# simonhmartin/genomics_general

Measured on NVIDIA H100. Metric: sites/sec popgenWindows (pi+Fst+Dxy), higher is better.
Workload: dtype u8

## Files before the change

genomics_general_b200/csrc/k1.cu:

```cuda
#include <stdlib.h>

#include <algorithm>
#include <climits>
#include <cmath>
#include <type_traits>
#include <cub/cub.cuh>

#include "pgwin_internal.h"

namespace {

constexpr int K1_MAX_WARPS = 12;

enum { MODE_POPGEN = 0, MODE_ABBA = 1, MODE_COUNTS = 2, MODE_POPGEN_FREQ = 3, MODE_FOURPOP = 4 };

struct K1Params {
    const uint8_t* geno;
    const int32_t* pos;
    int64_t site_begin, site_end;
    int64_t num_tiles;
    int pitch, G, I, T, wpt, stages, tile_bytes, nw;
    const int32_t* ent_chunk;
    const uint4* ent_mask;
    int n_ent;
// ... 822 lines not shown
        if (lane == 0) mbar_arrive(&empty[stage]);
    }
    if (MODE != MODE_COUNTS) flush();
}


template <int P>
__device__ __forceinline__ void packed_walk(const K1Params& prm, int G, int gsub, int sl, uint32_t (&walk)[P]) {
#pragma unroll
    for (int X = 0; X < P; ++X) {
        const int n = prm.ent_hi[X] - prm.ent_lo[X];
        const int cnt = gsub < n ? (n - gsub + G - 1) / G : 0;
        const int first = prm.ent_lo[X] + (n > 0 ? (((sl >> 2) & 7) + gsub) % n : 0);
        walk[X] = (uint32_t)first | ((uint32_t)cnt << 16);
    }
}

template <int P>
struct ArrCounts {
    uint32_t nn[P], cc[P][4];
    __device__ __forceinline__ void set(int X, uint32_t p0, uint32_t p1) {
        const uint32_t m = p0 & 0xffffu, n1 = p0 >> 16, n2 = p1 & 0xffffu, n3 = p1 >> 16;
        nn[X] = m;
        cc[X][0] = m - n1 - n2 + n3;
        cc[X][1] = n1 - n3;
        cc[X][2] = n2 - n3;
        cc[X][3] = n3;
    }
    __device__ __forceinline__ uint32_t n(int X) const { return nn[X]; }
    __device__ __forceinline__ uint32_t c(int X, int a) const { return cc[X][a]; }
};
template <int P>
struct PkCounts {
    uint32_t p0[P], p1[P];
    __device__ __forceinline__ void set(int X, uint32_t a, uint32_t b) {
        p0[X] = a;
        p1[X] = b;
    }
    __device__ __forceinline__ uint32_t n(int X) const { return p0[X] & 0xffffu; }
    __device__ __forceinline__ uint32_t c(int X, int a) const {
        const uint32_t n1 = p0[X] >> 16, n2 = p1[X] & 0xffffu, n3 = p1[X] >> 16;
        return a == 0 ? (p0[X] & 0xffffu) - n1 - n2 + n3 : (a == 1 ? n1 - n3 : (a == 2 ? n2 - n3 : n3));
    }
};

template <int P, class W, class CT>
__device__ __forceinline__ void packed_counts(const K1Params& prm, const uint2* s_ent, const uint32_t* row, const W& walk,
                                              int G, int spw, CT& ct) {
    const int wd = prm.wd;
#pragma unroll
    for (int X = 0; X < P; ++X) {
        uint32_t a = 0u, a1 = 0u, a2 = 0u, a3 = 0u;
        const int lo = prm.ent_lo[X], span = prm.ent_hi[X] - lo;
        int e = (int)(walk[X] & 0xffffu);
        const int cnt = (int)(walk[X] >> 16);
        for (int k = 0; k < cnt; ++k) {
            const uint2 em = s_ent[e];
            const uint32_t m = row[em.x] & em.y;
            const uint32_t b0 = row[wd + em.x], b1 = row[2 * wd + em.x];
            a += __popc(m);
            a1 += __popc(m & b0);
            a2 += __popc(m & b1);
            a3 += __popc(m & b0 & b1);
            e += G;
            if (e >= lo + span) e -= span;
        }
        uint32_t p0 = a | (a1 << 16), p1 = a2 | (a3 << 16);
        for (int d = spw; d < 32; d <<= 1) {
            p0 += __shfl_xor_sync(0xffffffffu, p0, d);
            p1 += __shfl_xor_sync(0xffffffffu, p1, d);
        }
        ct.set(X, p0, p1);
    }
}

template <int P, bool ONE, class CT>
__device__ __forceinline__ void varied_counts(const K1Params& prm, const uint2* s_ent, const uint32_t* row, int nvar, int Gv,
                                              int gsub, int spv, CT& ct) {
    const int pn = prm.wd * nvar;
#pragma unroll
    for (int X = 0; X < P; ++X) {
        uint32_t a = 0u, a1 = 0u, a2 = 0u, a3 = 0u;
#pragma unroll 1
        for (int e = prm.ent_lo[X] + (ONE ? 0 : gsub); e < prm.ent_hi[X]; e += (ONE ? 1 : Gv)) {
            const uint2 em = s_ent[e];
            const uint32_t* w = row + em.x * nvar;
            const uint32_t m = w[0] & em.y;
            const uint32_t b0 = w[pn], b1 = w[2 * pn];
            a += __popc(m);
            a1 += __popc(m & b0);
            a2 += __popc(m & b1);
            a3 += __popc(m & b0 & b1);
        }
        uint32_t p0 = a | (a1 << 16), p1 = a2 | (a3 << 16);
        for (int d = spv; !ONE && d < 32; d <<= 1) {
            p0 += __shfl_xor_sync(0xffffffffu, p0, d);
            p1 += __shfl_xor_sync(0xffffffffu, p1, d);
        }
        ct.set(X, p0, p1);
    }
}

template <int P>
struct BitCounts {
    uint32_t k[P];
    const int* N;
    __device__ __forceinline__ void set(int X, uint32_t kx) { k[X] = kx; }
    __device__ __forceinline__ uint32_t n(int X) const { return (uint32_t)N[X]; }
    __device__ __forceinline__ uint32_t c(int X, int a) const { return a == 0 ? (uint32_t)N[X] - k[X] : (a == 1 ? k[X] : 0u); }
};

__device__ __forceinline__ void bmma_and_popc(int (&d)[4], uint32_t a0, uint32_t a1, uint32_t a2, uint32_t a3, uint2 b) {
    asm("mma.sync.aligned.m16n8k256.row.col.s32.b1.b1.s32.and.popc {%0, %1, %2, %3}, {%4, %5, %6, %7}, {%8, %9}, "
        "{%0, %1, %2, %3};"
        : "+r"(d[0]), "+r"(d[1]), "+r"(d[2]), "+r"(d[3])
        : "r"(a0), "r"(a1), "r"(a2), "r"(a3), "r"(b.x), "r"(b.y));
}

__device__ __forceinline__ int mma_row(int lane) { return (lane >> 2) + 8 * (lane & 3); }

template <int P>
__device__ __forceinline__ void varied_mma(const uint2* s_bf, const uint32_t* rows, int n1, int wd, int r, int lane,
                                           BitCounts<P>& ct) {
    static_assert(P <= 4, "one-plane rows: up to 4 (padded) populations");
    const int g = lane >> 2, t = lane & 3;
    const int j0 = min(r + g, n1 - 1), j1 = min(r + g + 8, n1 - 1), j2 = min(r + g + 16, n1 - 1), j3 = min(r + g + 24, n1 - 1);
    int d0[4] = {0, 0, 0, 0}, d1[4] = {0, 0, 0, 0};
    const uint32_t* w = rows + t * n1;
    for (int kb = 0; kb * 8 < wd; ++kb, w += 8 * n1) {
        const bool lo = kb * 8 + t < wd, hi = kb * 8 + 4 + t < wd;
        const uint32_t* v = w + 4 * n1;
        const uint2 b = s_bf[kb * 32 + lane];
        bmma_and_popc(d0, lo ? w[j0] : 0u, lo ? w[j1] : 0u, hi ? v[j0] : 0u, hi ? v[j1] : 0u, b);
        bmma_and_popc(d1, lo ? w[j2] : 0u, lo ? w[j3] : 0u, hi ? v[j2] : 0u, hi ? v[j3] : 0u, b);
    }
    const uint32_t pk[4] = {(uint32_t)d0[0] | (uint32_t)d0[1] << 16, (uint32_t)d0[2] | (uint32_t)d0[3] << 16,
                            (uint32_t)d1[0] | (uint32_t)d1[1] << 16, (uint32_t)d1[2] | (uint32_t)d1[3] << 16};
    uint32_t k01 = 0u, k23 = 0u;
#pragma unroll
    for (int j = 0; j < 4; ++j) {
        const int q = t ^ j;
        const uint32_t v = __shfl_xor_sync(0xffffffffu, (q & 2) ? ((q & 1) ? pk[3] : pk[2]) : ((q & 1) ? pk[1] : pk[0]), j);
        if (q == 0) k01 = v;
        if (q == 1) k23 = v;
    }
    ct.set(0, k01 & 0xffffu);
    ct.set(1, k01 >> 16);
    if constexpr (P > 2) {
        ct.set(2, k23 & 0xffffu);
        ct.set(3, k23 >> 16);
    }
}

template <int P, class CT>
__device__ __forceinline__ void packed_class(const K1Params& prm, bool owner, const CT& ct, bool& pres, bool& ragged) {
    bool allpres = true, allmiss = true;
#pragma unroll
    for (int X = 0; X < P; ++X) {
        allpres = allpres && (ct.n(X) == (uint32_t)prm.popN[X]);
        allmiss = allmiss && (ct.n(X) == 0u);
    }
    pres = owner && allpres;
    ragged = owner && !allpres && !allmiss;
}

template <int MODE, int P, class ACC, class CT>
__device__ __forceinline__ void packed_add(ACC& acc, bool pres, bool ragged, const CT& ct) {
    acc.i[0] += pres ? 1 : 0;
    acc.i[1] += ragged ? 1 : 0;
    const uint32_t f = pres ? 1u : 0u;
#pragma unroll
    for (int X = 0; X < P; ++X) {
        const uint32_t sq = ct.c(X, 0) * ct.c(X, 0) + ct.c(X, 1) * ct.c(X, 1) + ct.c(X, 2) * ct.c(X, 2) + ct.c(X, 3) * ct.c(X, 3);
        acc.u[X] += sq * f;
        if (MODE == MODE_POPGEN_FREQ) acc.u[P + P * (P - 1) / 2 + X] += (pres && sq != ct.n(X) * ct.n(X)) ? 1u : 0u;
    }
    int k = 0;
#pragma unroll
    for (int X = 0; X < P; ++X)
#pragma unroll
        for (int Y = X + 1; Y < P; ++Y) {
            const uint32_t cr = ct.c(X, 0) * ct.c(Y, 0) + ct.c(X, 1) * ct.c(Y, 1) + ct.c(X, 2) * ct.c(Y, 2) + ct.c(X, 3) * ct.c(Y, 3);
            acc.u[P + k] += cr * f;
            ++k;
        }
}

template <int MODE, int P, int NW, bool UNI = false>
__global__ void __launch_bounds__((NW + 1) * 32, 1) k1_site_pass_packed(const __grid_constant__ K1Params prm) {
    static_assert(MODE == MODE_POPGEN || MODE == MODE_POPGEN_FREQ, "packed site pass: popgen modes");
    constexpr int K1_THREADS = (NW + 1) * 32;
    constexpr int QI = ModeTraits<MODE, P>::QI, QU = ModeTraits<MODE, P>::QU;
    extern __shared__ __align__(128) uint8_t smem[];
    uint8_t* tiles = smem;
    uint64_t* full = reinterpret_cast<uint64_t*>(smem + (size_t)prm.stages * prm.tile_bytes);
    uint64_t* empty = full + 8;
    volatile int* s_issued = reinterpret_cast<volatile int*>(empty + 8);
    volatile uint32_t* s_nvar = reinterpret_cast<volatile uint32_t*>(s_issued + 8);
    volatile long long* s_site0 = reinterpret_cast<volatile long long*>(s_issued + 16);
    uint2* s_ent = reinterpret_cast<uint2*>(smem + (size_t)prm.stages * prm.tile_bytes + 256);
    uint2* s_bf = s_ent + prm.n_ent;

    const int tid = threadIdx.x, lane = tid & 31, warp = tid >> 5;
    const int b = blockIdx.x, B = gridDim.x;
    const int64_t t0 = (int64_t)b * prm.num_tiles / B, t1 = (int64_t)(b + 1) * prm.num_tiles / B;
    const int ntiles = (int)(t1 - t0);

    for (int e = tid; e < prm.n_ent; e += K1_THREADS) s_ent[e] = prm.word_ent[e];
    if constexpr (UNI && P < 8)
        for (int e = tid; e < (prm.wd + 7) / 8 * 32; e += K1_THREADS) s_bf[e] = prm.bit_frag[e];
    const int Gv = prm.uni_gv > 0 ? prm.uni_gv : prm.G;
    if (tid == 0) {
        for (int s = 0; s < prm.stages; ++s) {
            mbar_init(&full[s], 1);
            mbar_init(&empty[s], (uint32_t)prm.wpt);
        }
        *s_issued = 0;
        asm volatile("fence.mbarrier_init.release.cluster;" ::: "memory");
        asm volatile("fence.proxy.async.shared::cta;" ::: "memory");
    }
    __syncthreads();

    if (warp == NW) {
        if (UNI) k1_producer_uniform(prm, tiles, full, empty, s_issued, s_nvar, s_site0, ntiles, t0, lane);
        else if (lane == 0) k1_producer<MODE>(prm, tiles, full, empty, s_issued, ntiles, t0);
        return;
    }

    const int nteams = NW / prm.wpt;
    const int team = warp / prm.wpt, lw = warp % prm.wpt;

    Acc<QI, QU, 0> acc;
#pragma unroll
    for (int q = 0; q < QI; ++q) acc.i[q] = 0;
#pragma unroll
    for (int q = 0; q < QU; ++q) acc.u[q] = 0u;
    int since_flush = 0;
    int cur_seg = -1;
    int64_t seg_end = -1;
    const int seg_first = prm.cta_seg_first[b];
    const int64_t slot_base = prm.cta_slot_off[b];

    if constexpr (!UNI) {
        const int G = prm.G;
        const int spw = 32 / G;
        const int gsub = lane / spw;
        const int sl = lane % spw;
        const int sites_per_iter = prm.wpt * spw;
        uint32_t walk[P];
        packed_walk<P>(prm, G, gsub, sl, walk);

        for (int it = team; it < ntiles; it += nteams) {
            const int stage = it % prm.stages;
            if (lane == 0)
                while (atomicAdd(const_cast<int*>(s_issued), 0) <= it) __nanosleep(20);
            __syncwarp();
            mbar_wait(&full[stage], (uint32_t)((it / prm.stages) & 1));
            const uint8_t* tile = tiles + (size_t)stage * prm.tile_bytes;
            const int64_t tile_site0 = prm.site_begin + (t0 + it) * prm.T;

            for (int i = 0; i < prm.I; ++i) {
                const int slot = i * sites_per_iter + lw * spw + sl;
                const int64_t site = tile_site0 + slot;
                const bool valid = site < prm.site_end;
                const bool owner = valid && (gsub == 0);
                const uint32_t* row = reinterpret_cast<const uint32_t*>(tile + (size_t)(valid ? slot : 0) * prm.pitch);
                const int posv = owner ? reinterpret_cast<const int32_t*>(tile + (size_t)prm.T * prm.pitch)[slot] : 0;

                ArrCounts<P> ct;
                packed_counts<P>(prm, s_ent, row, walk, G, spw, ct);

                int sg = cur_seg;
                if (owner && site >= seg_end) sg = find_seg(prm.brk, prm.nseg, cur_seg + 1, site);
                if (__any_sync(0xffffffffu, sg != cur_seg)) {
                    warp_flush<QI, QU, 0>(acc, cur_seg, prm.part, slot_base, seg_first, warp, lane, NW);
                    since_flush = 0;
                    if (sg != cur_seg) {
                        cur_seg = sg;
                        seg_end = __ldg(prm.brk + sg + 1);
                    }
                }
                bool pres, ragged;
                packed_class<P>(prm, owner, ct, pres, ragged);
                if (++since_flush > prm.acc_limit) {
                    warp_flush<QI, QU, 0>(acc, cur_seg, prm.part, slot_base, seg_first, warp, lane, NW);
                    since_flush = 1;
                }
                acc.i[2] += (long long)posv;
                packed_add<MODE, P>(acc, pres, ragged, ct);
            }

            __syncwarp();
            if (lane == 0) mbar_arrive(&empty[stage]);
        }
    } else {
        const int spv = 32 / Gv, gsub = lane / spv, sl = lane % spv, wpt = prm.wpt;
        auto add_row = [&](int64_t site, bool owner, const auto& ct, bool back) {
            int sg = cur_seg;
            if (owner && site >= seg_end) sg = next_seg(prm.brk, prm.nseg, cur_seg + 1, site);
            else if (back && owner && site < __ldg(prm.brk + cur_seg)) sg = find_seg(prm.brk, cur_seg, 0, site);
            if (__any_sync(0xffffffffu, sg != cur_seg)) {
                warp_flush<QI, QU, 0>(acc, cur_seg, prm.part, slot_base, seg_first, warp, lane, NW);
                since_flush = 0;
                const int last = __reduce_max_sync(0xffffffffu, sg);
                const int to = owner ? sg : last;
                if (to != cur_seg) {
                    cur_seg = to;
                    seg_end = __ldg(prm.brk + to + 1);
                }
            }
            bool pres, ragged;
            packed_class<P>(prm, owner, ct, pres, ragged);
            if (++since_flush > prm.acc_limit) {
                warp_flush<QI, QU, 0>(acc, cur_seg, prm.part, slot_base, seg_first, warp, lane, NW);
                since_flush = 1;
            }
            packed_add<MODE, P>(acc, pres, ragged, ct);
        };

        for (int it = team; it < ntiles; it += nteams) {
            const int stage = it % prm.stages;
            if (lane == 0)
                while (atomicAdd(const_cast<int*>(s_issued), 0) <= it) __nanosleep(20);
            __syncwarp();
            mbar_wait(&full[stage], (uint32_t)((it / prm.stages) & 1));
            const uint8_t* tile = tiles + (size_t)stage * prm.tile_bytes;
            const int64_t tile_site0 = s_site0[stage];
            const uint32_t sizes = s_nvar[stage];
            const int n1 = (int)(sizes & 0xffffu), n3 = (int)(sizes >> 16);
            const uint16_t* s_slot = reinterpret_cast<const uint16_t*>(tile + (size_t)prm.row_cap * prm.pitch);
            const int rot = (int)((t0 + it) % wpt), nb1 = (n1 + 31) / 32;

            if constexpr (P < 8) {
                for (int r = ((lw - rot + wpt) % wpt) * 32; r < n1; r += wpt * 32) {
                    const int rw = r + mma_row(lane);
                    BitCounts<P> ct;
                    ct.N = prm.popN;
                    varied_mma<P>(s_bf, reinterpret_cast<const uint32_t*>(tile), n1, prm.wd, r, lane, ct);
                    add_row(tile_site0 + (rw < n1 ? s_slot[rw] : 0), rw < n1, ct, false);
                }
            }

            const uint32_t* rows3 = reinterpret_cast<const uint32_t*>(tile) + ((n1 * prm.wd + 3) & ~3);
            for (int r = ((lw - rot - nb1 % wpt + 2 * wpt) % wpt) * spv; r < n3; r += wpt * spv) {
                const int rw = r + sl;
                const bool valid = rw < n3;
                const bool owner = valid && (gsub == 0);
                const uint32_t* row = rows3 + (valid ? rw : r);
                std::conditional_t<P == 8, ArrCounts<P>, PkCounts<P>> ct;
                if (P < 8 && Gv == 1) varied_counts<P, true>(prm, s_ent, row, n3, 1, 0, 32, ct);
                else varied_counts<P, false>(prm, s_ent, row, n3, Gv, gsub, spv, ct);
                add_row(tile_site0 + (valid ? s_slot[n1 + rw] : 0), owner, ct, true);
            }

            __syncwarp();
            if (lane == 0) mbar_arrive(&empty[stage]);
        }
    }
    warp_flush<QI, QU, 0>(acc, cur_seg, prm.part, slot_base, seg_first, warp, lane, NW);
}

struct FinParams {
    const unsigned long long* part;
    const int32_t* seg_cta_lo;
    const int32_t* seg_cta_hi;
    const int32_t* cta_seg_first;
    const int64_t* cta_slot_off;
    const int32_t* win_seg_lo;
    const int32_t* win_seg_hi;
    const int64_t* win_lo;
    const int64_t* win_hi;
    int64_t W;
    int Q, QI, nw;
    int P;
    int Ppad;
    int popN[PG_MAX_K1_POPS];
    double harm_a[PG_MAX_K1_POPS], harm_a2[PG_MAX_K1_POPS];
    int min_sites;
    double min_data;
    int force_path;
    int with_freq;
    int bookkeeping_only;
    const int64_t* pre_pos;
    const int64_t* pre_uni;
    int64_t S;
    unsigned long long* rec;
    int RC;
    int32_t* path;
    int* n_pairwise;
};

__device__ __forceinline__ unsigned long long d2u(double x) { return (unsigned long long)__double_as_longlong(x); }

__device__ __forceinline__ double nan_d() { return __longlong_as_double(0x7ff8000000000000ll); }

__device__ __forceinline__ double cf_pi(long long N, long long Lp, long long sumsq, bool all_nan, double min_data) {
    if (N <= 0) return nan_d();
    const double size = (double)(N * N);
    const double nan_cnt = all_nan ? size : (double)N;
    if (1.0 - (1.0 * nan_cnt / size) < min_data) return nan_d();
    if (all_nan) return nan_d();
    const double num = (double)(N * N * Lp - sumsq);
    const double den = (double)((N * N - N) * Lp);
    return num / den;
}

template <int MODE>
__global__ void __launch_bounds__(64) k1_finalize(const __grid_constant__ FinParams fp) {
    __shared__ unsigned long long sums[64];
    const int q = threadIdx.x;
    for (int64_t w = blockIdx.x; w < fp.W; w += gridDim.x) {
        __syncthreads();
        if (q < fp.Q) {
            long long si = 0;
            double sd = 0.0;
            for (int g = fp.win_seg_lo[w]; g < fp.win_seg_hi[w]; ++g) {
                for (int b = fp.seg_cta_lo[g]; b <= fp.seg_cta_hi[g]; ++b) {
                    const unsigned long long* src =
                        fp.part + fp.cta_slot_off[b] + (int64_t)(g - fp.cta_seg_first[b]) * fp.nw * fp.Q;
                    for (int wp = 0; wp < fp.nw; ++wp) {
                        const unsigned long long v = src[wp * fp.Q + q];
                        if (q < fp.QI) si += (long long)v; else sd += __longlong_as_double((long long)v);
                    }
                }
            }
            if (MODE == MODE_POPGEN && fp.pre_uni) {
                const int64_t lo = min(max(fp.win_lo[w], (int64_t)0), fp.S), hi = min(max(fp.win_hi[w], lo), fp.S);
                const long long u = fp.pre_uni[hi] - fp.pre_uni[lo];
                const int Pp = fp.Ppad;
                if (q == 0) si += u;
                else if (q == 2) si += fp.pre_pos[hi] - fp.pre_pos[lo];
                else if (q >= 3 && q < 3 + Pp + Pp * (Pp - 1) / 2) {
                    int X = q - 3, Y = X;
                    if (X >= Pp) {
                        int k = X - Pp, left = Pp - 1;
                        for (X = 0; k >= left; ++X, --left) k -= left;
                        Y = X + 1 + k;
                    }
                    si += u * (long long)fp.popN[X] * (long long)fp.popN[Y];
                }
            }
            sums[q] = (q < fp.QI) ? (unsigned long long)si : (unsigned long long)__double_as_longlong(sd);
        }
        __syncthreads();
        if (q != 0) continue;
        const long long sites = fp.win_hi[w] - fp.win_lo[w];
        unsigned long long* rec = fp.rec + (size_t)w * fp.RC;
        rec[0] = (unsigned long long)sites;
        rec[1] = sums[2];
        if (MODE == MODE_POPGEN) {
            const int P = fp.P, Pp = fp.Ppad;
            const int npairs = P * (P - 1) / 2;
            double* pi_o = reinterpret_cast<double*>(rec + 3);
            double* dxy_o = pi_o + P;
            double* fst_o = dxy_o + npairs;
            const long long Lp = (long long)sums[0];
            const bool ragged = (long long)sums[1] > 0;
            if (fp.bookkeeping_only) {
                const int path = sites < fp.min_sites ? 0 : 2;
                fp.path[w] = path;
                rec[2] = (unsigned long long)path;
                if (path == 2) atomicAdd(fp.n_pairwise, 1);
                for (int k = 3; k < fp.RC; ++k) rec[k] = d2u(nan_d());
                continue;
            }
            {
                double* fq = fst_o + npairs;
                fq[0] = fp.with_freq ? (double)Lp : nan_d();
                const int npp = Pp * (Pp - 1) / 2;
                for (int x = 0; x < P; ++x) {
                    double Sx = nan_d(), tpi = nan_d(), tw = nan_d(), tD = nan_d();
                    if (Lp >= 1 && fp.with_freq) {
                        const long long N = fp.popN[x];
                        const long long seg = (long long)sums[3 + Pp + npp + x];
                        const long long pairs = (N * N * Lp - (long long)sums[3 + x]) / 2;
                        Sx = (double)seg;
                        tpi = (double)pairs / (.5 * (double)N * (double)(N - 1));
                        const double a = fp.harm_a[x], a2 = fp.harm_a2[x];
                        tw = (double)seg / a;
                        const double n_ = (double)N;
                        const double b1 = (n_ + 1.) / (3 * (n_ - 1));
                        const double b2 = (2. * (n_ * n_ + n_ + 3)) / (9 * n_ * (n_ - 1));
                        const double c1 = b1 - (1. / a);
                        const double c2 = b2 - ((n_ + 2) / (a * n_)) + a2 / (a * a);
                        const double e1 = c1 / a;
                        const double e2 = c2 / (a * a + a2);
                        const double d = tpi - tw;
                        tD = d / sqrt(e1 * Sx + e2 * Sx * (Sx - 1));
                    }
                    fq[1 + x] = Sx;
                    fq[1 + P + x] = tpi;
                    fq[1 + 2 * P + x] = tw;
                    fq[1 + 3 * P + x] = tD;
                }
            }
            int path = 1;
            if (sites < fp.min_sites) path = 0;
            else if (ragged || fp.force_path == 2) path = 2;
            fp.path[w] = path;
            rec[2] = (unsigned long long)path;
            if (path == 2) atomicAdd(fp.n_pairwise, 1);
            if (path != 1) {
                for (int x = 0; x < P; ++x) pi_o[x] = nan_d();
                for (int k = 0; k < npairs; ++k) dxy_o[k] = fst_o[k] = nan_d();
                continue;
            }
            const bool all_nan = (Lp == 0) || (fp.min_sites > 0 && Lp < fp.min_sites);
            double piv[PG_MAX_K1_POPS];
            for (int x = 0; x < P; ++x) {
                piv[x] = cf_pi(fp.popN[x], Lp, (long long)sums[3 + x], all_nan, fp.min_data);
// ... 441 lines not shown
        cta_seg_last[b] = g1;
        off += (int64_t)(g1 - g0 + 1) * nw * Q;
    }
    for (int g = 0; g < nseg; ++g) {
        L.seg_cta_lo[g] = B;
        L.seg_cta_hi[g] = -1;
    }
    for (int b = 0; b < B; ++b) {
        if (cta_seg_last[b] < 0) continue;
        for (int g = L.cta_seg_first[b]; g <= cta_seg_last[b]; ++g) {
            L.seg_cta_lo[g] = std::min(L.seg_cta_lo[g], b);
            L.seg_cta_hi[g] = std::max(L.seg_cta_hi[g], b);
        }
    }
    L.words = off;
}

int push_slots(pg_ctx* ctx, uint8_t* base, size_t& o, const HostSlots& h, SlotTables& st) {
    PG_TRY(push(ctx, base, o, h.cta_seg_first.data(), h.cta_seg_first.size(), &st.cta_seg_first));
    PG_TRY(push(ctx, base, o, h.cta_slot_off.data(), h.cta_slot_off.size(), &st.cta_slot_off));
    PG_TRY(push(ctx, base, o, h.seg_cta_lo.data(), h.seg_cta_lo.size(), &st.seg_cta_lo));
    PG_TRY(push(ctx, base, o, h.seg_cta_hi.data(), h.seg_cta_hi.size(), &st.seg_cta_hi));
    st.words = h.words;
    return PG_OK;
}

void fill_params(K1Params& p, const pg_ctx* ctx, const K1Plan& pl, const PopTables& pt, const DevTables& dt, bool packed) {
    memset(&p, 0, sizeof(p));
    p.geno = packed ? (const uint8_t*)ctx->d_packed : (const uint8_t*)ctx->d_geno;
    p.pos = ctx->d_pos;
    p.num_tiles = pl.num_tiles;
    p.pitch = pl.pitch;
    p.G = pl.G;
    p.I = pl.I;
    p.T = pl.T;
    p.wpt = pl.wpt;
    p.nw = pl.nw;
    p.stages = pl.stages;
    p.tile_bytes = pl.tile_bytes;
    p.ent_chunk = dt.ent_chunk;
    p.ent_mask = dt.ent_mask;
    p.word_ent = dt.word_ent;
    p.bit_frag = dt.bit_frag;
    p.wd = (ctx->H + 31) / 32;
    p.n_ent = packed ? (int)pt.word_ent.size() / 2 : (int)pt.ent_chunk.size();
    for (int X = 0; X < PG_MAX_K1_POPS; ++X) {
        p.ent_lo[X] = pt.ent_lo[X];
        p.ent_hi[X] = pt.ent_hi[X];
        p.full_lo[X] = pt.full_lo[X];
        p.full_hi[X] = pt.full_hi[X];
        p.popN[X] = pt.popN[X];
    }
}

int prepare_windowed(pg_ctx* ctx, K1Cache& c, const std::vector<int32_t>& hap_pop_local, int Ppad, int Q, int nw, int force_G,
                     bool packed) {
    K1Launch& L = c.L;
    DevTables& dt = c.dt;
    PopTables& pt = c.pt;
    PG_TRY(pg_build_segments(ctx));
    if (packed) {
        build_word_tables(hap_pop_local, ctx->H, Ppad, pt);
        const int table_bytes = table_bytes_of(pt);
        PG_CHECK(table_bytes <= 48 * 1024, "population layout needs %d bytes of mask tables (limit 48 KiB)", table_bytes);
        L.plan = pg_make_k1_plan_rows(ctx->S, ctx->packed_pitch, ctx->sm_count, table_bytes, nw, force_G);
        PG_CHECK(L.plan.stages >= 2, "rows of %d haplotypes are too long for the packed site pass (%d bytes)", ctx->H,
                 L.plan.pitch);
        PG_TRY(check_plan(L.plan));
    } else {
        PG_TRY(byte_plan(ctx, hap_pop_local, Ppad, nw, force_G, pt, L.plan));
    }
    for (int X = 0; X < Ppad; ++X) PG_CHECK(pt.popN[X] <= 65535, "a population has more than 65535 haplotypes");
    const K1Plan& pl = L.plan;
    const int B = pl.ctas;
    std::vector<int64_t> bound(B + 1);
    for (int b = 0; b <= B; ++b) bound[b] = std::min<int64_t>((int64_t)b * pl.num_tiles / B * pl.T, ctx->S);
    HostSlots hs;
    slot_tables(ctx->brk, bound, nw, Q, hs);
    size_t bytes = 4096 + pt.ent_mask.size() * 4 + pt.ent_chunk.size() * 4 + pt.word_ent.size() * 4 + pt.bit_frag.size() * 4 +
                   ctx->brk.size() * 8 + hs.bytes() + (size_t)ctx->W * 24 + 14 * 16;
    PG_TRY(c.tables.ensure(bytes));
    uint8_t* base = (uint8_t*)c.tables.p;
    size_t o = 0;
    uint32_t* d_mask_words = nullptr;
    PG_TRY(push(ctx, base, o, pt.ent_mask.data(), pt.ent_mask.size(), &d_mask_words));
    dt.ent_mask = reinterpret_cast<uint4*>(d_mask_words);
    PG_TRY(push(ctx, base, o, pt.ent_chunk.data(), pt.ent_chunk.size(), &dt.ent_chunk));
    uint32_t* d_word_ent = nullptr;
    PG_TRY(push(ctx, base, o, pt.word_ent.data(), pt.word_ent.size(), &d_word_ent));
    dt.word_ent = reinterpret_cast<uint2*>(d_word_ent);
    uint32_t* d_bit_frag = nullptr;
    PG_TRY(push(ctx, base, o, pt.bit_frag.data(), pt.bit_frag.size(), &d_bit_frag));
    dt.bit_frag = reinterpret_cast<uint2*>(d_bit_frag);
    PG_TRY(push(ctx, base, o, ctx->brk.data(), ctx->brk.size(), &dt.brk));
    PG_TRY(push_slots(ctx, base, o, hs, L.slots));
    PG_TRY(push(ctx, base, o, ctx->win_seg_lo.data(), ctx->win_seg_lo.size(), &dt.win_seg_lo));
    PG_TRY(push(ctx, base, o, ctx->win_seg_hi.data(), ctx->win_seg_hi.size(), &dt.win_seg_hi));
    PG_TRY(push(ctx, base, o, ctx->win_lo.data(), ctx->win_lo.size(), &dt.win_lo));
    PG_TRY(push(ctx, base, o, ctx->win_hi.data(), ctx->win_hi.size(), &dt.win_hi));
    PG_CHECK(o <= c.tables.cap, "internal: table buffer overflow");
    PG_CUDA(cudaStreamSynchronize(ctx->stream));

    K1Params& p = L.prm;
    fill_params(p, ctx, pl, pt, dt, packed);
    p.site_begin = 0;
    p.site_end = ctx->S;
    p.brk = dt.brk;
    p.nseg = (int)ctx->brk.size() - 1;
    p.cta_seg_first = L.slots.cta_seg_first;
    p.cta_slot_off = L.slots.cta_slot_off;
    return PG_OK;
}

int arm_slots(pg_ctx* ctx, K1Launch& L, const void* rows) {
    const size_t bytes = (size_t)std::max<int64_t>(L.slots.words, 1) * 8;
    PG_TRY(ctx->part.ensure(bytes));
    PG_CUDA(cudaMemsetAsync(ctx->part.p, 0, bytes, ctx->stream));
    L.prm.part = (unsigned long long*)ctx->part.p;
    L.prm.geno = (const uint8_t*)rows;
    L.prm.pos = ctx->d_pos;
    return PG_OK;
}

template <auto Kern, int NW>
int launch_kernel(pg_ctx* ctx, const K1Launch& L, const char* name) {
    PG_TRY(pg_smem_limit<Kern>(ctx, 227 * 1024));
    const int ti = pg_time_begin(ctx, name);
    Kern<<<L.plan.ctas, (NW + 1) * 32, L.plan.smem_bytes, ctx->stream>>>(L.prm);
    pg_time_end(ctx, ti);
    PG_CUDA(cudaGetLastError());
    return PG_OK;
}

template <int MODE, int P>
int launch_site_pass(pg_ctx* ctx, const K1Launch& L, const char* name) {
    constexpr bool POPGEN_MODE = (MODE == MODE_POPGEN || MODE == MODE_POPGEN_FREQ);
    const bool w12 = L.prm.nw == 12;
    if constexpr ((POPGEN_MODE || MODE == MODE_COUNTS) && (P == 4 || P == 8)) {
        if (L.prm.lanepop)
            return w12 ? launch_kernel<k1_site_pass_lp<MODE, P, 12>, 12>(ctx, L, name)
                       : launch_kernel<k1_site_pass_lp<MODE, P, 8>, 8>(ctx, L, name);
    }
    if constexpr (POPGEN_MODE) {
        if (L.prm.bytes)
            return w12 ? launch_kernel<k1_site_pass<MODE, P, 12, true>, 12>(ctx, L, name)
                       : launch_kernel<k1_site_pass<MODE, P, 8, true>, 8>(ctx, L, name);
    }
    return w12 ? launch_kernel<k1_site_pass<MODE, P, 12, false>, 12>(ctx, L, name)
               : launch_kernel<k1_site_pass<MODE, P, 8, false>, 8>(ctx, L, name);
}

template <int MODE, int P, bool UNI>
int launch_site_pass_packed(pg_ctx* ctx, const K1Launch& L, const char* name) {
    return L.prm.nw == 12 ? launch_kernel<k1_site_pass_packed<MODE, P, 12, UNI>, 12>(ctx, L, name)
                          : launch_kernel<k1_site_pass_packed<MODE, P, 8, UNI>, 8>(ctx, L, name);
}

template <typename F>
int with_pops(int Pp, F&& f) {
    if (Pp == 2) return f(std::integral_constant<int, 2>());
    if (Pp == 4) return f(std::integral_constant<int, 4>());
    return f(std::integral_constant<int, 8>());
}

template <typename F>
int with_popgen_mode(bool with_freq, int Pp, F&& f) {
    return with_pops(Pp, [&](auto P) {
        return with_freq ? f(std::integral_constant<int, MODE_POPGEN_FREQ>(), P) : f(std::integral_constant<int, MODE_POPGEN>(), P);
    });
}

constexpr double UNI_MIN_FRACTION = 0.125;

int uni_word_rows(int R, int pitch, int wd) { return (R * (pitch / 4) - 3) / wd; }

int uni_stage_bytes(int row_cap, int cap_rows, int pitch) {
    return (int)align_up((size_t)row_cap * pitch + align_up((size_t)cap_rows * 2, 16), 128);
}

void uni_geometry(UniformPass& u) {
    const K1Plan& pl = u.plan;
    const char* eb = getenv("PG_K1_UNI_BITS");
    u.bits = u.one_plane && !(eb && *eb && atoi(eb) == 0);
    const char* er = getenv("PG_K1_UNI_R");
    u.words = u.bits && !(er && *er);
    int Tmax = u.words ? 2048 : 512;
    if (const char* e = getenv("PG_K1_UNI_TMAX")) Tmax = std::max(8, std::min(32768, (atoi(e) + 7) / 8 * 8));
    const int lanes = 32 / std::max(1, pl.G);
    int R = lanes * pl.wpt;
    auto stage = [&](int r) {
        const bool w = u.words && r >= 2;
        u.row_cap = w ? r + 1 : r;
        u.cap_rows = w ? uni_word_rows(r, pl.pitch, u.wd) : r;
        return uni_stage_bytes(u.row_cap, u.cap_rows, pl.pitch);
    };
    if (er && *er) {
        R = std::max(1, std::min(0x7fff, atoi(er)));
    } else {
        while (R > lanes && pg_k1_ring_stages(stage(R), u.table_bytes) < 2) R /= 2;
    }
    u.words = u.words && R >= 2;
    u.R = R;
    u.Tmax = Tmax;
    u.stage_bytes = stage(R);
    u.stages = pl.stages >= 2 ? pg_k1_ring_stages(u.stage_bytes, u.table_bytes) : 0;
}

int uniform_prepare(pg_ctx* ctx, UniformPass& u) {
    UniformStream& us = u.us;
    const bool forced = getenv("PG_K1_UNIFORM_FORCE") != nullptr;
    const bool bits = u.bits, wb = u.words;
    const int R = u.R, Tmax = u.Tmax;
    if (us.gen == ctx->data_gen && us.R == R && us.Tmax == Tmax && us.forced == forced && us.bits == bits && us.wb == wb)
        return PG_OK;
    us.wb = wb;
    us.gen = ctx->data_gen;
    us.R = R;
    us.Tmax = Tmax;
    us.forced = forced;
    us.bits = bits;
    us.in_use = false;
    us.varied = ctx->S;
    us.serial += 1;
    if (u.stages < 2) return PG_OK;
    const int64_t S = ctx->S;
    constexpr int CH = 2048;
    const int64_t nc = (S + CH - 1) / CH;
    const int ppw = ctx->packed_pitch / 4, wd = u.wd;
    const int64_t Bw = (int64_t)u.cap_rows * wd;
    const int64_t nt_max = S / Tmax + 1 + (wb ? S * ppw / Bw + 2 : (S + R - 1) / R) + 1;
    const int64_t nscan = std::max(nc, nt_max) + 1;
    PG_TRY(us.cnt.ensure((size_t)nscan * 8));
    PG_TRY(us.row0.ensure((size_t)nscan * 8));
    int64_t* d_cnt = (int64_t*)us.cnt.p;
    int64_t* d_row0 = (int64_t*)us.row0.p;
    size_t scan_bytes = 0, pre_bytes = 0;
    PG_CUDA(cub::DeviceScan::ExclusiveSum(nullptr, scan_bytes, d_cnt, d_row0, nscan, ctx->stream));
    const auto uni_in = cub::TransformInputIterator<int64_t, UniformSite, const uint8_t*>(ctx->d_site_cls, UniformSite());
    const auto pos_in = cub::TransformInputIterator<int64_t, Widen, const int32_t*>(ctx->d_pos, Widen());
    PG_CUDA(cub::DeviceScan::ExclusiveSum(nullptr, pre_bytes, uni_in, d_row0, S + 1, ctx->stream));
    PG_TRY(us.scan.ensure(std::max(scan_bytes, pre_bytes)));
    int ti = pg_time_begin(ctx, "k1_uniform");
    PG_CUDA(cudaMemsetAsync(d_cnt + nc, 0, 8, ctx->stream));
    k1_uni_count<<<(unsigned)nc, 256, 0, ctx->stream>>>(ctx->d_site_cls, S, nullptr, CH, d_cnt);
    PG_CUDA(cudaGetLastError());
    PG_CUDA(cub::DeviceScan::ExclusiveSum(us.scan.p, scan_bytes, d_cnt, d_row0, nc + 1, ctx->stream));
    pg_time_end(ctx, ti);
    int64_t varied = 0;
    PG_CUDA(cudaMemcpyAsync(&varied, d_row0 + nc, 8, cudaMemcpyDeviceToHost, ctx->stream));
    PG_CUDA(cudaStreamSynchronize(ctx->stream));
    us.varied = varied;
    if (!forced && (double)(S - varied) < UNI_MIN_FRACTION * (double)S) return PG_OK;
    int64_t ng = varied > 0 ? (wb ? varied * ppw / Bw + 2 : (varied + R - 1) / R) : 1;
    if (us.slots.ensure((size_t)nt_max * Tmax * 2) != PG_OK || us.src.ensure((size_t)std::max<int64_t>(varied, 1) * 8) != PG_OK ||
        us.rows.ensure((size_t)std::max<int64_t>(varied, 1) * ctx->packed_pitch + (size_t)nt_max * 16) != PG_OK ||
        us.site_lo.ensure((size_t)(nt_max + 1) * 8) != PG_OK || us.groups.ensure((size_t)(ng + 1) * 8 * 2) != PG_OK ||
        us.info.ensure((size_t)(ctx->sm_count + 2) * 8) != PG_OK || us.words.ensure((size_t)(nt_max + 1) * 8 * 2) != PG_OK ||
        us.n1.ensure((size_t)(nt_max + 1) * 4) != PG_OK || us.pre.ensure((size_t)(S + 1) * 8 * 2) != PG_OK ||
        (wb && us.wts.ensure((size_t)(varied + 1) * 8 * 2 + (size_t)(ng + 1) * 8) != PG_OK)) {
        cudaGetLastError();
        for (PgBuf* b : {&us.rows, &us.src, &us.slots, &us.pre}) b->release();
        return PG_OK;
    }
    int64_t* d_src = (int64_t*)us.src.p;
    int64_t* d_pieces = (int64_t*)us.groups.p;
    int64_t* d_base = d_pieces + ng + 1;
    int64_t* d_site_lo = (int64_t*)us.site_lo.p;
    int64_t* d_info = (int64_t*)us.info.p;
    int64_t* d_wcnt = (int64_t*)us.words.p;
    int64_t* d_woff = d_wcnt + nt_max + 1;
    us.woff = d_woff;
    int32_t* d_n1 = (int32_t*)us.n1.p;
    int64_t* d_pre = (int64_t*)us.pre.p;
    ti = pg_time_begin(ctx, "k1_uniform");
    k1_uni_rows<<<(unsigned)nc, 256, 0, ctx->stream>>>(ctx->d_site_cls, S, nullptr, CH, d_row0, d_src);
    PG_CUDA(cudaGetLastError());
    int64_t* d_first = nullptr;
    if (wb && varied > 0) {
        int64_t* w = (int64_t*)us.wts.p;
        int64_t* cw = w + varied + 1;
        d_first = cw + varied + 1;
        k1_uni_w<<<ctx->sm_count * 8, 256, 0, ctx->stream>>>(ctx->d_site_cls, d_src, varied, wd, ppw, bits, w);
        PG_CUDA(cudaGetLastError());
        size_t tb = 0;
        PG_CUDA(cub::DeviceScan::ExclusiveSum(nullptr, tb, w, cw, varied + 1, ctx->stream));
        PG_TRY(us.scan2.ensure(tb));
        PG_CUDA(cub::DeviceScan::ExclusiveSum(us.scan2.p, tb, w, cw, varied + 1, ctx->stream));
        k1_uni_first<<<ctx->sm_count * 8, 256, 0, ctx->stream>>>(cw, varied, Bw, d_first);
        PG_CUDA(cudaGetLastError());
        int64_t last = 0;
        PG_CUDA(cudaMemcpyAsync(&last, cw + varied - 1, 8, cudaMemcpyDeviceToHost, ctx->stream));
        PG_CUDA(cudaStreamSynchronize(ctx->stream));
        ng = last / Bw + 1;
    } else if (wb) {
        ng = 1;
    }
    PG_CUDA(cudaMemsetAsync(d_pieces + ng, 0, 8, ctx->stream));
    k1_uni_groups<<<(unsigned)((ng + 255) / 256), 256, 0, ctx->stream>>>(d_src, R, S, Tmax, ng, d_pieces, d_first);
    PG_CUDA(cudaGetLastError());
    PG_CUDA(cub::DeviceScan::ExclusiveSum(us.scan.p, scan_bytes, d_pieces, d_base, ng + 1, ctx->stream));
    const int64_t nfill = std::max(ng, nt_max) + 1;
    k1_uni_tiles<<<(unsigned)std::min<int64_t>((nfill + 255) / 256, (int64_t)ctx->sm_count * 16), 256, 0, ctx->stream>>>(
        d_src, R, S, Tmax, ng, d_base, nt_max, d_site_lo, d_first);
    PG_CUDA(cudaGetLastError());
    PG_CUDA(cudaMemsetAsync(d_cnt + nt_max, 0, 8, ctx->stream));
    PG_CUDA(cudaMemsetAsync(d_wcnt + nt_max, 0, 8, ctx->stream));
// ... 1281 lines not shown
```

Before: 62.38 billion.

## Accumulate varied-row pair statistics via u8 IMMA Gram matrix instead of per-site adds

Adds a GRAM variant of the packed site pass for the uniform-ploidy byte path with up to 4 populations. Per-site allele counts from the binary MMA are packed into bytes and fed to an m16n8k32 u8 tensor-core MMA, so the within- and between-population sums of squares accumulate as a Gram matrix across rows. The pi/Dxy sums are then reconstructed algebraically at segment flush instead of using per-lane scalar multiply-add per site. It adds segment-boundary ballot handling and periodic flushes to avoid overflow, and risks correctness subtleties in the algebra and lane mapping.

```diff
diff --git a/genomics_general_b200/csrc/k1.cu b/genomics_general_b200/csrc/k1.cu
--- a/genomics_general_b200/csrc/k1.cu
+++ b/genomics_general_b200/csrc/k1.cu
@@ -998,6 +998,38 @@
     }
 }
 
+__device__ __forceinline__ void gram_counts(const uint2* s_bf, const uint32_t* rows, int n1, int wd, int r, int lane,
+                                            uint32_t& k0, uint32_t& k1) {
+    const int g = lane >> 2, t = lane & 3, j = r + g;
+    const bool v0 = j < n1, v1 = j + 8 < n1, v2 = j + 16 < n1, v3 = j + 24 < n1;
+    int d[4][4] = {{0, 0, 0, 0}, {0, 0, 0, 0}, {0, 0, 0, 0}, {0, 0, 0, 0}};
+    const uint32_t* w = rows + t * n1 + j;
+    for (int kb = 0; kb * 8 < wd; ++kb, w += 8 * n1) {
+        const bool lo = kb * 8 + t < wd, hi = kb * 8 + 4 + t < wd;
+        const uint32_t* v = w + 4 * n1;
+        const uint2 a = s_bf[kb * 32 + lane];
+        bmma_and_popc(d[0], a.x, 0u, a.y, 0u, make_uint2(lo && v0 ? w[0] : 0u, hi && v0 ? v[0] : 0u));
+        bmma_and_popc(d[1], a.x, 0u, a.y, 0u, make_uint2(lo && v1 ? w[8] : 0u, hi && v1 ? v[8] : 0u));
+        bmma_and_popc(d[2], a.x, 0u, a.y, 0u, make_uint2(lo && v2 ? w[16] : 0u, hi && v2 ? v[16] : 0u));
+        bmma_and_popc(d[3], a.x, 0u, a.y, 0u, make_uint2(lo && v3 ? w[24] : 0u, hi && v3 ? v[24] : 0u));
+    }
+    k0 = (uint32_t)d[0][0] | (uint32_t)d[0][1] << 8 | (uint32_t)d[1][0] << 16 | (uint32_t)d[1][1] << 24;
+    k1 = (uint32_t)d[2][0] | (uint32_t)d[2][1] << 8 | (uint32_t)d[3][0] << 16 | (uint32_t)d[3][1] << 24;
+}
+
+__device__ __forceinline__ uint32_t gram_bytes(uint32_t m, int t, int half) {
+    const uint32_t x = m >> (2 * t + 16 * half);
+    const uint32_t b = (x & 3u) | ((x >> 6) & 0xcu);
+    return ((b * 0x00204081u) & 0x01010101u) * 0xffu;
+}
+
+__device__ __forceinline__ void imma_u8(int (&d)[2], uint32_t a0, uint32_t a2, uint32_t b0, uint32_t b1) {
+    int z0, z1;
+    asm("mma.sync.aligned.m16n8k32.row.col.s32.u8.u8.s32 {%0, %1, %2, %3}, {%4, %5, %6, %7}, {%8, %9}, {%0, %1, %10, %10};"
+        : "+r"(d[0]), "+r"(d[1]), "=r"(z0), "=r"(z1)
+        : "r"(a0), "r"(0u), "r"(a2), "r"(0u), "r"(b0), "r"(b1), "r"(0));
+}
+
 template <int P, class CT>
 __device__ __forceinline__ void packed_class(const K1Params& prm, bool owner, const CT& ct, bool& pres, bool& ragged) {
     bool allpres = true, allmiss = true;
@@ -1032,9 +1064,10 @@
         }
 }
 
-template <int MODE, int P, int NW, bool UNI = false>
+template <int MODE, int P, int NW, bool UNI = false, bool GRAM = false>
 __global__ void __launch_bounds__((NW + 1) * 32, 1) k1_site_pass_packed(const __grid_constant__ K1Params prm) {
     static_assert(MODE == MODE_POPGEN || MODE == MODE_POPGEN_FREQ, "packed site pass: popgen modes");
+    static_assert(!GRAM || (UNI && P <= 4), "the Gram of the one-plane rows: varied-row stream, up to 4 (padded) populations");
     constexpr int K1_THREADS = (NW + 1) * 32;
     constexpr int QI = ModeTraits<MODE, P>::QI, QU = ModeTraits<MODE, P>::QU;
     extern __shared__ __align__(128) uint8_t smem[];
@@ -1164,6 +1197,66 @@
             packed_add<MODE, P>(acc, pres, ragged, ct);
         };
 
+        int gseg = -1, grows = 0;
+        int64_t gseg_end = -1;
+        int gd[2] = {0, 0};
+        uint32_t gfreq = 0u;
+        const uint32_t gN4 = (lane >> 2) < P ? (uint32_t)prm.popN[min(lane >> 2, P - 1)] * 0x01010101u : 0u;
+        const int glimit = max(prm.acc_limit / 2, 32);
+        auto gram_flush = [&]() {
+            if (grows == 0) return;
+            __syncwarp();
+            int X = 0, Y = 0;
+            long long NX = 0, NY = 0;
+            int k = P;
+#pragma unroll
+            for (int x = 0; x < P; ++x) {
+                if (lane == x || lane == P + P * (P - 1) / 2 + x) X = Y = x;
+#pragma unroll
+                for (int y = x + 1; y < P; ++y, ++k)
+                    if (lane == k) {
+                        X = x;
+                        Y = y;
+                    }
+            }
+#pragma unroll
+            for (int x = 0; x < P; ++x) {
+                if (X == x) NX = prm.popN[x];
+                if (Y == x) NY = prm.popN[x];
+            }
+            const int src = 4 * X + (Y >> 1);
+            const int d0 = __shfl_sync(0xffffffffu, gd[0], src), d1 = __shfl_sync(0xffffffffu, gd[1], src);
+            const long long SX = __shfl_sync(0xffffffffu, gd[0], 4 * X + 2);
+            const long long SY = __shfl_sync(0xffffffffu, gd[0], 4 * Y + 2);
+            const long long n = __shfl_sync(0xffffffffu, gd[0], 18);
+            uint32_t f = gfreq;
+            f += __shfl_xor_sync(0xffffffffu, f, 1);
+            f += __shfl_xor_sync(0xffffffffu, f, 2);
+            f = __shfl_sync(0xffffffffu, f, 4 * X);
+            unsigned long long* dst = prm.part + slot_base + ((int64_t)(gseg - seg_first) * NW + warp) * (QI + QU);
+            if (lane < P + P * (P - 1) / 2)
+                dst[QI + lane] += (unsigned long long)(n * NX * NY - NX * SY - NY * SX + 2ll * ((Y & 1) ? d1 : d0));
+            else if (lane < QU)
+                dst[QI + lane] += (unsigned long long)f;
+            else if (lane == 31)
+                dst[0] += (unsigned long long)n;
+            __syncwarp();
+            gd[0] = gd[1] = 0;
+            gfreq = 0u;
+            grows = 0;
+        };
+        auto gram_add = [&](uint32_t k0, uint32_t k1, uint32_t m) {
+            if (grows + __popc(m) > glimit) gram_flush();
+            grows += __popc(m);
+            const int t = lane & 3;
+            if ((lane >> 2) == 4) k0 = k1 = 0x01010101u;
+            k0 &= gram_bytes(m, t, 0);
+            k1 &= gram_bytes(m, t, 1);
+            imma_u8(gd, k0, k1, k0, k1);
+            if (MODE == MODE_POPGEN_FREQ)
+                gfreq += __popc((__vsetgtu4(k0, 0u) & __vsetltu4(k0, gN4)) | (__vsetgtu4(k1, 0u) & __vsetltu4(k1, gN4)) << 1);
+        };
+
         for (int it = team; it < ntiles; it += nteams) {
             const int stage = it % prm.stages;
             if (lane == 0)
@@ -1177,7 +1270,30 @@
             const uint16_t* s_slot = reinterpret_cast<const uint16_t*>(tile + (size_t)prm.row_cap * prm.pitch);
             const int rot = (int)((t0 + it) % wpt), nb1 = (n1 + 31) / 32;
 
-            if constexpr (P < 8) {
+            if constexpr (GRAM) {
+                for (int r = ((lw - rot + wpt) % wpt) * 32; r < n1; r += wpt * 32) {
+                    uint32_t k0, k1;
+                    gram_counts(s_bf, reinterpret_cast<const uint32_t*>(tile), n1, prm.wd, r, lane, k0, k1);
+                    const int nv = min(32, n1 - r);
+                    uint32_t pending = nv == 32 ? 0xffffffffu : (1u << nv) - 1u;
+                    if (tile_site0 + s_slot[r + nv - 1] < gseg_end) {
+                        gram_add(k0, k1, pending);
+                        continue;
+                    }
+                    const int64_t site = tile_site0 + s_slot[r + min(lane, nv - 1)];
+                    while (pending) {
+                        const int64_t first = __shfl_sync(0xffffffffu, site, __ffs(pending) - 1);
+                        if (first >= gseg_end) {
+                            gram_flush();
+                            gseg = next_seg(prm.brk, prm.nseg, gseg + 1, first);
+                            gseg_end = __ldg(prm.brk + gseg + 1);
+                        }
+                        const uint32_t in = pending & __ballot_sync(0xffffffffu, site < gseg_end);
+                        gram_add(k0, k1, in);
+                        pending &= ~in;
+                    }
+                }
+            } else if constexpr (P < 8) {
                 for (int r = ((lw - rot + wpt) % wpt) * 32; r < n1; r += wpt * 32) {
                     const int rw = r + mma_row(lane);
                     BitCounts<P> ct;
@@ -1202,6 +1318,7 @@
             __syncwarp();
             if (lane == 0) mbar_arrive(&empty[stage]);
         }
+        if constexpr (GRAM) gram_flush();
     }
     warp_flush<QI, QU, 0>(acc, cur_seg, prm.part, slot_base, seg_first, warp, lane, NW);
 }
@@ -1949,6 +2066,11 @@
 
 template <int MODE, int P, bool UNI>
 int launch_site_pass_packed(pg_ctx* ctx, const K1Launch& L, const char* name) {
+    if constexpr (UNI && P < 8) {
+        if (L.prm.bytes)
+            return L.prm.nw == 12 ? launch_kernel<k1_site_pass_packed<MODE, P, 12, true, true>, 12>(ctx, L, name)
+                                  : launch_kernel<k1_site_pass_packed<MODE, P, 8, true, true>, 8>(ctx, L, name);
+    }
     return L.prm.nw == 12 ? launch_kernel<k1_site_pass_packed<MODE, P, 12, UNI>, 12>(ctx, L, name)
                           : launch_kernel<k1_site_pass_packed<MODE, P, 8, UNI>, 8>(ctx, L, name);
 }
```

Result: faster. 70.23 billion, median of 6 (+12.6%).
